# GATECH-EIC/BNS-GCN

Measured on AMD Instinct MI355X. Metric: training throughput (full-graph edges/s), reddit-shaped graphsage 3-layer h=256, sampling-rate=0.1, higher is better.
Workload: dtype fp32; 1 GPU; model=graphsage, dataset=reddit, n_layers=3, n_hidden=256, n_nodes=232965, n_edges=114756398, use_pp=True, partition=metis, parallelism=partition-parallel p1

## Files before the change

### bnsgcn_amd/models/context.py

```python
from __future__ import annotations

import torch

from ..graph.store import Partition
from ..ops.csr_torch import transpose_csr, merge_csr
from ..parallel.halo import partition_aggregate
from ..parallel.plan import EpochState, HaloPlan


def _inv_sqrt(x: torch.Tensor) -> torch.Tensor:
    return 1.0 / torch.sqrt(x.clamp_min(1.0))


def _inv(x: torch.Tensor) -> torch.Tensor:
    return 1.0 / x.clamp_min(1.0)


class GraphContext:
    def __init__(self, indptr, indices, in_deg, out_deg, device,
                 plan: HaloPlan | None = None, need_eperm: bool = True):
        dev = torch.device(device)
        self.plan = plan
        self.indptr = indptr.to(dev)
        self.indices = indices.to(dev)
        tip, tix, t_eperm = transpose_csr(self.indptr, self.indices,
                                          n_cols=self.indptr.numel() - 1
                                          if plan is None else plan.n_inner)
        self.t_indptr, self.t_indices = tip, tix
        self.t_eperm = t_eperm if need_eperm else None
        self.loss_rows: torch.Tensor | None = None
        self._rows_static: tuple | None = None
        self._rows_halo: tuple | None = None
        in_deg = in_deg.to(dev).float()
        out_deg = out_deg.to(dev).float()
        self.in_norm_inv = _inv_sqrt(in_deg)
        self.out_norm_inv = _inv_sqrt(out_deg)
        self.in_deg_inv = _inv(in_deg)
        self.n_rows = self.indptr.numel() - 1
        if dev.type == "cuda":
            from ..ops.functional import _worklist_of
            _worklist_of(self.indptr)
            _worklist_of(self.t_indptr)
        self._gat_cache: tuple[int, tuple] | None = None
        self._full_state: EpochState | None = None

    @classmethod
    def for_partition(cls, part: Partition, plan: HaloPlan, device,
                      need_eperm: bool = True) -> "GraphContext":
        return cls(torch.from_numpy(part.inner_indptr),
                   torch.from_numpy(part.inner_indices),
                   torch.from_numpy(part.in_deg),
                   torch.from_numpy(part.out_deg), device, plan=plan,
                   need_eperm=need_eperm)

    @classmethod
    def for_full_graph(cls, csr_indptr, csr_indices, in_deg, out_deg, device
                       ) -> "GraphContext":
        return cls(csr_indptr, csr_indices, in_deg, out_deg, device, plan=None)

    @property
    def inner_csrs(self):
        return (self.indptr, self.indices, self.t_indptr, self.t_indices)

    def aggregate(self, x: torch.Tensor, mode: str,
                  rows: torch.Tensor | None = None) -> torch.Tensor:
        if mode == "gcn":
            src, dst, halo_src = self.out_norm_inv, self.in_norm_inv, True
        elif mode == "mean":
            src, dst, halo_src = None, self.in_deg_inv, False
        else:
            raise ValueError(mode)
        if rows is not None:
            dst = dst[rows]
        if self.plan is None:
            from ..ops.functional import spmm_sum
            if rows is None:
                return spmm_sum(x, *self.inner_csrs, src_scale=src,
                                dst_scale=dst)
            ip, ix, tip, tix = self._rows_inner_csrs(rows)
            return spmm_sum(x, ip, ix, tip, tix, src_scale=src, dst_scale=dst)
        if rows is None:
            return partition_aggregate(x, self.plan, self.inner_csrs, src,
                                       dst, halo_src)
        import dataclasses
        st = self.plan.state
        hfip, hfix, hbip, hbix = self._rows_halo_csrs(rows, st)
        st_r = dataclasses.replace(st, halo_fwd_indptr=hfip,
                                   halo_fwd_indices=hfix,
                                   halo_bwd_indptr=hbip,
                                   halo_bwd_indices=hbix)
        ip, ix, tip, tix = self._rows_inner_csrs(rows)
        from ..parallel.halo import _PartitionAggregate
        return _PartitionAggregate.apply(x, self.plan, st_r, ip, ix, tip, tix,
                                         src, dst, halo_src)

    def _rows_inner_csrs(self, rows: torch.Tensor):
        from ..ops.csr_torch import gather_rows_csr
        if self._rows_static is None:
            ip, ix = gather_rows_csr(self.indptr, self.indices, rows)
            n_src = self.n_rows if self.plan is None else self.plan.n_inner
            tip, tix, _ = transpose_csr(ip, ix, n_src)
            if self.indptr.is_cuda:
                from ..ops.functional import _worklist_of
                _worklist_of(ip)
                _worklist_of(tip)
            self._rows_static = (ip, ix, tip, tix)
        return self._rows_static

    def _rows_halo_csrs(self, rows: torch.Tensor, st: EpochState):
        if self._rows_halo is not None and self._rows_halo[0] == st.epoch:
            ev = self._rows_halo[2]
            if ev is not None:
                cur = torch.cuda.current_stream()
                cur.wait_event(ev)
                for t in self._rows_halo[1]:
                    t.record_stream(cur)
                    wl = getattr(t, "_bns_worklist", None)
                    if wl is not None:
                        for w in wl:
                            w.record_stream(cur)
                self._rows_halo = (st.epoch, self._rows_halo[1], None)
            return self._rows_halo[1]
        out = self._build_rows_halo(rows, st)
        self._rows_halo = (st.epoch, out, None)
        return out
# ... 135 lines not shown
```

### bnsgcn_amd/ops/csr_torch.py

```python
from __future__ import annotations

import torch


def row_lengths(indptr: torch.Tensor) -> torch.Tensor:
    return indptr[1:] - indptr[:-1]


def transpose_csr(indptr: torch.Tensor, indices: torch.Tensor, n_cols: int
                  ) -> tuple[torch.Tensor, torch.Tensor, torch.Tensor]:
    device = indices.device
    n_rows = indptr.numel() - 1
    row = torch.repeat_interleave(torch.arange(n_rows, device=device, dtype=indices.dtype),
                                  row_lengths(indptr))
    eperm = torch.argsort(indices.long(), stable=True)
    indices_t = row[eperm]
    sorted_cols = indices[eperm]
    bounds = torch.arange(n_cols + 1, device=device, dtype=sorted_cols.dtype)
    indptr_t = torch.searchsorted(sorted_cols, bounds).to(indptr.dtype)
    return indptr_t, indices_t, eperm


import os

SEG = int(os.environ.get("BNSGCN_SEG", 512))
MAX_WAVES = int(os.environ.get("BNSGCN_MAX_WAVES", 131072))


def build_worklist(indptr: torch.Tensor, seg: int = None, max_waves: int = None
                   ) -> tuple[torch.Tensor, torch.Tensor, torch.Tensor, torch.Tensor]:
    seg = seg or SEG
    max_waves = max_waves or MAX_WAVES
    device = indptr.device
    deg = (indptr[1:] - indptr[:-1])
    n = deg.numel()
    nseg = torch.clamp((deg + (seg - 1)) // seg, min=1)
    total = int(nseg.sum())
    rows = torch.repeat_interleave(torch.arange(n, device=device), nseg)
    item_first = torch.cumsum(nseg, 0)
    item_first = torch.cat([torch.zeros(1, dtype=item_first.dtype, device=device),
                            item_first[:-1]])
    k = torch.arange(total, device=device) - item_first[rows]
    wbeg = indptr[rows] + k * seg
    wend = torch.minimum(wbeg + seg, indptr[rows + 1])
    split = nseg[rows] > 1
    wrow = torch.where(split, ~rows, rows).to(torch.int32)

    empty_rows = torch.nonzero(deg == 0, as_tuple=True)[0]
    atomic_rows = torch.nonzero(nseg > 1, as_tuple=True)[0]
    zero_rows = torch.cat([empty_rows, atomic_rows])
    keep = wend > wbeg
    wrow, wbeg, wend = wrow[keep], wbeg[keep], wend[keep]
    total = int(keep.sum())
    if total == 0:
        z = torch.zeros(0, dtype=torch.int32, device=device)
        return (z, wbeg, wend, torch.zeros(1, dtype=torch.int32, device=device),
                zero_rows)

    lens = (wend - wbeg)
    cum = torch.cumsum(torch.cat([torch.zeros(1, dtype=lens.dtype, device=device),
                                  lens]), 0)
    if total >= 1_000_000:
        max_waves = max(max_waves, 262144)
    n_waves = min(max_waves, max(8, total))
    n_waves = (n_waves + 7) // 8 * 8
    targets = (cum[-1] * torch.arange(n_waves + 1, device=device).double()
               / n_waves).to(cum.dtype)
    wave_start = torch.searchsorted(cum, targets).to(torch.int32)
    wave_start[0] = 0
    wave_start[-1] = total
    return (wrow.contiguous(), wbeg.contiguous(), wend.contiguous(),
            wave_start.contiguous(), zero_rows)


def merge_csr(ip1: torch.Tensor, ix1: torch.Tensor,
              ip2: torch.Tensor, ix2: torch.Tensor,
              col_offset2: int) -> tuple[torch.Tensor, torch.Tensor]:
    device = ix1.device
    n = ip1.numel() - 1
    l1 = row_lengths(ip1)
    l2 = row_lengths(ip2)
    ip = torch.zeros(n + 1, dtype=ip1.dtype, device=device)
    torch.cumsum(l1 + l2, 0, out=ip[1:])
    ix = torch.empty(int(ip[-1]), dtype=ix1.dtype, device=device)
    rows = torch.arange(n, device=device)
    if ix1.numel():
        r1 = torch.repeat_interleave(rows, l1)
        e1 = torch.arange(ix1.numel(), device=device)
        ix[ip[r1] + (e1 - ip1[r1])] = ix1
    if ix2.numel():
        r2 = torch.repeat_interleave(rows, l2)
        e2 = torch.arange(ix2.numel(), device=device)
        ix[ip[r2] + l1[r2] + (e2 - ip2[r2])] = (ix2 + col_offset2).to(ix1.dtype)
    return ip, ix


def gather_rows_csr(indptr: torch.Tensor, indices: torch.Tensor,
                    rows: torch.Tensor) -> tuple[torch.Tensor, torch.Tensor]:
    device = indices.device
    lens = row_lengths(indptr)[rows]
    new_indptr = torch.zeros(rows.numel() + 1, dtype=indptr.dtype, device=device)
    torch.cumsum(lens, 0, out=new_indptr[1:])
    total = int(new_indptr[-1])
    if total == 0:
        return new_indptr, torch.zeros(0, dtype=indices.dtype, device=device)
    starts = indptr[rows]
    pos = torch.arange(total, device=device)
    row_of_new_edge = torch.repeat_interleave(
        torch.arange(rows.numel(), device=device), lens)
    offset_in_row = pos - new_indptr[row_of_new_edge]
    src_edge = starts[row_of_new_edge] + offset_in_row
    return new_indptr, indices[src_edge]
```

### bnsgcn_amd/ops/functional.py

```python
from __future__ import annotations

import torch
from torch.autograd import Function

from . import reference as ref
from ._ext import get_ext, use_hip



def _worklist_of(indptr):
    wl = getattr(indptr, "_bns_worklist", None)
    if wl is None:
        from .csr_torch import build_worklist
        wl = build_worklist(indptr)
        indptr._bns_worklist = wl
    return wl


def spmm_sum_raw(indptr, indices, x, src_scale=None, dst_scale=None, out=None):
    if use_hip(x):
        wrow, wbeg, wend, wave_start, zero_rows = _worklist_of(indptr)
        acc = out is not None
        if not acc:
            out = torch.empty(indptr.numel() - 1, x.shape[1],
                              dtype=x.dtype, device=x.device)
            if zero_rows.numel():
                out.index_fill_(0, zero_rows, 0.0)
        return get_ext().spmm_sum(wrow, wbeg, wend, wave_start, indices, x,
                                  src_scale, dst_scale, out, acc)
    return ref.spmm_sum(indptr, indices, x, src_scale, dst_scale, out)


def spmm_edge_raw(indptr, indices, eweight, x, out=None, wperm=None):
    if use_hip(x):
        wrow, wbeg, wend, wstart, zero_rows = _worklist_of(indptr)
        acc = out is not None
        if not acc:
            out = torch.empty(indptr.numel() - 1, x.shape[1], x.shape[2],
                              dtype=x.dtype, device=x.device)
            if zero_rows.numel():
                out.index_fill_(0, zero_rows, 0.0)
        return get_ext().spmm_edge_sum(wrow, wbeg, wend, wstart, indptr,
                                       indices, eweight.contiguous(), wperm,
                                       x.contiguous(), out, acc)
    ew = eweight if wperm is None else eweight[wperm]
    return ref.spmm_edge_sum(indptr, indices, ew, x, out)


def sddmm_dot_raw(indptr, indices, a_dst, b_src):
    if use_hip(a_dst):
        wl = _worklist_of(indptr)[:4]
        return get_ext().sddmm_dot(*wl, indptr, indices,
                                   a_dst.contiguous(), b_src.contiguous())
    return ref.sddmm_dot(indptr, indices, a_dst, b_src)


def sddmm_add_raw(indptr, indices, el_src, er_dst, slope=-1.0):
    if use_hip(el_src):
        wl = _worklist_of(indptr)[:4]
        return get_ext().sddmm_add(*wl, indptr, indices,
                                   el_src.contiguous(), er_dst.contiguous(),
                                   slope)
    out = ref.sddmm_add(indptr, indices, el_src, er_dst)
    if slope >= 0:
        out = torch.nn.functional.leaky_relu(out, slope)
    return out


def segment_softmax_raw(indptr, logits):
    if use_hip(logits):
        return get_ext().segment_softmax(indptr, logits)
    return ref.segment_softmax(indptr, logits)


def segment_softmax_bwd_raw(indptr, alpha, grad_alpha):
    if use_hip(alpha):
        return get_ext().segment_softmax_backward(indptr, alpha, grad_alpha)
    return ref.segment_softmax_backward(indptr, alpha, grad_alpha)


def pack_rows_raw(x, idx, scale=None):
    if use_hip(x):
        return get_ext().pack_rows(x, idx, scale)
    return ref.pack_rows(x, idx, scale)


def scatter_add_rows_raw(out, idx, src, scale=None):
    if use_hip(out):
        get_ext().scatter_add_rows(out, idx, src, scale)
        return out
    return ref.scatter_add_rows(out, idx, src, scale)



class _SpMMSum(Function):

    @staticmethod
    def forward(ctx, x, indptr, indices, indptr_t, indices_t, src_scale, dst_scale):
        ctx.save_for_backward(indptr_t, indices_t, src_scale, dst_scale)
        return spmm_sum_raw(indptr, indices, x, src_scale, dst_scale)

    @staticmethod
    def backward(ctx, grad):
# ... 58 lines not shown
            gx_h = spmm_edge_raw(hbip, hbix, w_h, grad, wperm=heperm_t)
        if ctx.needs_input_grad[3]:
            gw_h = sddmm_dot_raw(hip_, hix_, grad, x_h)
        return (gx_in, gw_in, gx_h, gw_h) + (None,) * 10


def spmm_edge_sum2(x_in, w_in, x_h, w_h, inner_csrs5, halo_csrs5):
    return _SpMMEdge2.apply(x_in, w_in, x_h, w_h,
                            *inner_csrs5, *halo_csrs5)


class _SDDMMAdd(Function):

    @staticmethod
    def forward(ctx, el, er, indptr, indices, indptr_t, indices_t, eperm_t,
                slope):
        out = sddmm_add_raw(indptr, indices, el, er,
                            -1.0 if slope is None else float(slope))
        ctx.slope = slope
        if slope is not None:
            ctx.save_for_backward(indptr, indices, indptr_t, indices_t,
                                  eperm_t, out)
        else:
            ctx.save_for_backward(indptr, indices, indptr_t, indices_t,
                                  eperm_t)
        ctx.n_src, ctx.n_dst = el.shape[0], er.shape[0]
        return out

    @staticmethod
    def backward(ctx, grad):
        if ctx.slope is not None:
            indptr, indices, indptr_t, indices_t, eperm_t, out = ctx.saved_tensors
            grad = torch.where(out > 0, grad, grad * ctx.slope).contiguous()
        else:
            indptr, indices, indptr_t, indices_t, eperm_t = ctx.saved_tensors
            grad = grad.contiguous()
        g_el = g_er = None
        if use_hip(grad) and grad.shape[1] <= 8:
            e = get_ext()
            if ctx.needs_input_grad[0]:
                g_el = e.segment_sum_edges(*_worklist_of(indptr_t)[:4], eperm_t,
                                           grad, ctx.n_src)
            if ctx.needs_input_grad[1]:
                g_er = e.segment_sum_edges(*_worklist_of(indptr)[:4], None,
                                           grad, ctx.n_dst)
            return g_el, g_er, None, None, None, None, None, None
        if ctx.needs_input_grad[0]:
            g_el = torch.zeros(ctx.n_src, grad.shape[1], dtype=grad.dtype,
                               device=grad.device)
            g_el.index_add_(0, indices.long(), grad)
        if ctx.needs_input_grad[1]:
            g_er = torch.zeros(ctx.n_dst, grad.shape[1], dtype=grad.dtype,
                               device=grad.device)
            row = torch.repeat_interleave(
                torch.arange(ctx.n_dst, device=grad.device),
                indptr[1:] - indptr[:-1])
            g_er.index_add_(0, row, grad)
        return g_el, g_er, None, None, None, None, None, None


def sddmm_add(el, er, indptr, indices, indptr_t, indices_t, eperm_t,
              slope=None):
    return _SDDMMAdd.apply(el, er, indptr, indices, indptr_t, indices_t,
                           eperm_t, slope)


class _SegmentSoftmax(Function):
    @staticmethod
    def forward(ctx, logits, indptr):
        alpha = segment_softmax_raw(indptr, logits)
        ctx.save_for_backward(alpha, indptr)
        return alpha

    @staticmethod
    def backward(ctx, grad):
        alpha, indptr = ctx.saved_tensors
        return segment_softmax_bwd_raw(indptr, alpha, grad.contiguous()), None


def segment_softmax(logits, indptr):
    return _SegmentSoftmax.apply(logits, indptr)


import os as _os

_GEMM_MODE = _os.environ.get("BNSGCN_GEMM", "auto")


class _Linear(Function):

    @staticmethod
    def forward(ctx, x, weight, bias):
        ctx.save_for_backward(x, weight)
        ctx.has_bias = bias is not None
        if use_hip(x) and _GEMM_MODE == "hip":
            return get_ext().gemm_nt_bias(x, weight, bias)
        return torch.nn.functional.linear(x, weight, bias)

    @staticmethod
    def backward(ctx, grad):
        x, weight = ctx.saved_tensors
        grad = grad.contiguous()
        gx = gw = gb = None
        if use_hip(x):
            e = get_ext()
            if ctx.needs_input_grad[0]:
                gx = e.gemm_nn(grad, weight) if _GEMM_MODE == "hip" \
                    else grad @ weight
            if ctx.needs_input_grad[1]:
                gw = e.gemm_tn(grad, x)
            if ctx.has_bias and ctx.needs_input_grad[2]:
                return gx, gw, e.syncbn_stats(grad)[0]
        else:
            if ctx.needs_input_grad[0]:
                gx = grad @ weight
            if ctx.needs_input_grad[1]:
                gw = grad.t() @ x
        if ctx.has_bias and ctx.needs_input_grad[2]:
            gb = grad.sum(0)
        return gx, gw, gb


def linear(x, weight, bias=None):
    return _Linear.apply(x, weight, bias)


class _DropoutLinear(Function):

    @staticmethod
    def forward(ctx, x, weight, bias, keep, seed):
        x = x.contiguous()
        ctx.save_for_backward(x, weight)
        ctx.keep, ctx.seed = keep, seed
        ctx.has_bias = bias is not None
        return get_ext().gemm_nt_bias_drop(x, weight.contiguous(), bias,
                                           keep, seed)

    @staticmethod
    def backward(ctx, grad):
        x, weight = ctx.saved_tensors
        grad = grad.contiguous()
        e = get_ext()
        gw = gb = None
        if ctx.needs_input_grad[1]:
            gw = e.gemm_tn_drop(grad, x, ctx.keep, ctx.seed)
        if ctx.has_bias and ctx.needs_input_grad[2]:
            gb = e.syncbn_stats(grad)[0]
        return None, gw, gb, None, None


def dropout_linear(x, weight, bias, p: float, training: bool):
    if (training and p > 0.0 and use_hip(x) and x.dtype == torch.float32
            and not x.requires_grad):
        seed = int(torch.randint(0, 2**62, (1,)).item())
        return _DropoutLinear.apply(x, weight, bias, 1.0 - p, seed)
    return linear(dropout(x, p, training), weight, bias)


class _BiasAdd(Function):

    @staticmethod
    def forward(ctx, h, bias):
        return h + bias

    @staticmethod
    def backward(ctx, grad):
        gb = None
        if ctx.needs_input_grad[1]:
# ... 140 lines not shown
```

### bnsgcn_amd/ops/hip/kernels.hip

```cpp
#include <hip/hip_runtime.h>
#include <torch/extension.h>
#include <ATen/cuda/CUDAContext.h>
#include <c10/util/Optional.h>
#include <algorithm>
#include "common.h"
#include "gemm_tiled.h"

namespace {


DEV_INLINE void f4_axpy(float4& a, float ss, const float4 v) {
  a.x += ss * v.x; a.y += ss * v.y; a.z += ss * v.z; a.w += ss * v.w;
}

template <bool ACC, int SUBW>
__global__ __launch_bounds__(256) void spmm_sum_vec4_kernel(
    const int32_t* __restrict__ wrow, const int64_t* __restrict__ wbeg,
    const int64_t* __restrict__ wend, const int32_t* __restrict__ wave_start,
    const int32_t* __restrict__ indices, const float* __restrict__ x,
    const float* __restrict__ src_scale, const float* __restrict__ dst_scale,
    float* __restrict__ out, int f4) {
  const WorkList wl = {wrow, wbeg, wend, wave_start};
  const WaveItems wi = wave_items<SUBW>(wl);
  const int lane = wi.lane;
  const float4* __restrict__ x4 = reinterpret_cast<const float4*>(x);
  float4* __restrict__ out4 = reinterpret_cast<float4*>(out);

  for (int it = wi.beg; it < wi.end; ++it) {
    const WorkItem wk = work_item(wl, it);
    const float ds = dst_scale ? dst_scale[wk.row] : 1.0f;
    for (int f0 = 0; f0 < f4; f0 += 2 * SUBW) {
      const int fA = f0 + lane;
      const int fB = fA + SUBW;
      const bool hasA = fA < f4, hasB = fB < f4;
      float4 acc0 = {0.f, 0.f, 0.f, 0.f}, acc1 = {0.f, 0.f, 0.f, 0.f};
      for (int64_t e0 = wk.beg; e0 < wk.end; e0 += SUBW) {
        const Chunk ch = load_chunk<SUBW>(indices, src_scale, e0, wk.end, lane);
#pragma unroll 4
        for (int k = 0; k < ch.nv; ++k) {
          const int c = __shfl(ch.cid, k, SUBW);
          const float ss = src_scale ? __shfl(ch.ssc, k, SUBW) : 1.0f;
          const int64_t base = (int64_t)c * f4;
          if (hasA) f4_axpy(acc0, ss, x4[base + fA]);
          if (hasB) f4_axpy(acc1, ss, x4[base + fB]);
        }
      }
      const int64_t ob = (int64_t)wk.row * f4;
      if (hasA) store_row<ACC>(&out4[ob + fA], acc0, wk.atomic, ds);
      if (hasB) store_row<ACC>(&out4[ob + fB], acc1, wk.atomic, ds);
    }
  }
}

template <bool ACC, int G>
__global__ __launch_bounds__(256) void spmm_sum_narrow_kernel(
    const int32_t* __restrict__ wrow, const int64_t* __restrict__ wbeg,
    const int64_t* __restrict__ wend, const int32_t* __restrict__ wave_start,
    const int32_t* __restrict__ indices, const float* __restrict__ x,
    const float* __restrict__ src_scale, const float* __restrict__ dst_scale,
    float* __restrict__ out, int f4) {
  constexpr int NG = WAVE / G;
  const WorkList wl = {wrow, wbeg, wend, wave_start};
  const WaveItems wi = wave_items<WAVE>(wl);
  const int lane = wi.lane;
  const int g = lane / G, j = lane % G;
  const bool has = j < f4;
  const float4* __restrict__ x4 = reinterpret_cast<const float4*>(x);
  float4* __restrict__ out4 = reinterpret_cast<float4*>(out);

  for (int it = wi.beg; it < wi.end; ++it) {
    const WorkItem wk = work_item(wl, it);
    const float ds = dst_scale ? dst_scale[wk.row] : 1.0f;
    float4 acc = {0.f, 0.f, 0.f, 0.f};
    for (int64_t e0 = wk.beg; e0 < wk.end; e0 += WAVE) {
      const Chunk ch = load_chunk<WAVE>(indices, src_scale, e0, wk.end, lane);
#pragma unroll 4
      for (int k = 0; k < ch.nv; k += NG) {
        const int kk = k + g;
        const int c = __shfl(ch.cid, kk, WAVE);
        const float ss = src_scale ? __shfl(ch.ssc, kk, WAVE) : 1.0f;
        if (has && kk < ch.nv) f4_axpy(acc, ss, x4[(int64_t)c * f4 + j]);
      }
    }
#pragma unroll
    for (int off = G; off < WAVE; off <<= 1) {
      acc.x += __shfl_xor(acc.x, off, WAVE);
      acc.y += __shfl_xor(acc.y, off, WAVE);
      acc.z += __shfl_xor(acc.z, off, WAVE);
      acc.w += __shfl_xor(acc.w, off, WAVE);
    }
    if (g == 0 && has)
      store_row<ACC>(&out4[(int64_t)wk.row * f4 + j], acc, wk.atomic, ds);
  }
}

template <bool ACC>
__global__ __launch_bounds__(256) void spmm_sum_vec2_kernel(
    const int32_t* __restrict__ wrow, const int64_t* __restrict__ wbeg,
    const int64_t* __restrict__ wend, const int32_t* __restrict__ wave_start,
    const int32_t* __restrict__ indices, const float* __restrict__ x,
    const float* __restrict__ src_scale, const float* __restrict__ dst_scale,
    float* __restrict__ out, int f2) {
  const WorkList wl = {wrow, wbeg, wend, wave_start};
  const WaveItems wi = wave_items<WAVE>(wl);
  const int lane = wi.lane;
  const float2* __restrict__ x2 = reinterpret_cast<const float2*>(x);
  float2* __restrict__ out2 = reinterpret_cast<float2*>(out);
  for (int it = wi.beg; it < wi.end; ++it) {
    const WorkItem wk = work_item(wl, it);
    const float ds = dst_scale ? dst_scale[wk.row] : 1.0f;
    for (int f0 = 0; f0 < f2; f0 += 4 * WAVE) {
      float2 acc[4] = {{0.f, 0.f}, {0.f, 0.f}, {0.f, 0.f}, {0.f, 0.f}};
      for (int64_t e0 = wk.beg; e0 < wk.end; e0 += WAVE) {
        const Chunk ch = load_chunk<WAVE>(indices, src_scale, e0, wk.end, lane);
#pragma unroll 4
        for (int k = 0; k < ch.nv; ++k) {
          const int c = __shfl(ch.cid, k, WAVE);
          const float ss = src_scale ? __shfl(ch.ssc, k, WAVE) : 1.0f;
          const int64_t base = (int64_t)c * f2;
#pragma unroll
          for (int j = 0; j < 4; ++j) {
            const int f = f0 + j * WAVE + lane;
            if (f < f2) {
              const float2 v = x2[base + f];
              acc[j].x += ss * v.x;
              acc[j].y += ss * v.y;
            }
          }
        }
      }
      const int64_t ob = (int64_t)wk.row * f2;
#pragma unroll
// ... 1119 lines not shown
}

int env_int(const char* name, int dflt) {
  const char* e = getenv(name);
  return e ? atoi(e) : dflt;
}

struct WorkListArgs {
  WorkList wl;
  int n_waves;
};

WorkListArgs worklist_args(const at::Tensor& wrow, const at::Tensor& wbeg,
                           const at::Tensor& wend,
                           const at::Tensor& wave_start) {
  TORCH_CHECK(wrow.scalar_type() == at::kInt &&
                  wbeg.scalar_type() == at::kLong &&
                  wend.scalar_type() == at::kLong &&
                  wave_start.scalar_type() == at::kInt,
              "worklist: wrow/wave_start int32 and wbeg/wend int64 expected");
  for (const at::Tensor* t : {&wrow, &wbeg, &wend, &wave_start})
    TORCH_CHECK(t->is_cuda() && t->is_contiguous() &&
                    t->device() == wave_start.device(),
                "worklist arrays must be contiguous CUDA tensors on one "
                "device");
  TORCH_CHECK(wave_start.numel() >= 1 && wbeg.numel() == wrow.numel() &&
                  wend.numel() == wrow.numel(),
              "worklist: inconsistent array lengths (wrow ", wrow.numel(),
              ", wbeg ", wbeg.numel(), ", wend ", wend.numel(),
              ", wave_start ", wave_start.numel(), ")");
  const int n_waves = (int)wave_start.numel() - 1;
  TORCH_CHECK(n_waves % 8 == 0, "worklist: n_waves (", n_waves,
              ") must be a multiple of 8");
  return {{wrow.data_ptr<int32_t>(), wbeg.data_ptr<int64_t>(),
           wend.data_ptr<int64_t>(), wave_start.data_ptr<int32_t>()},
          n_waves};
}

template <typename K, typename... Args>
void launch_worklist(K kernel, const WorkListArgs& w, int subw,
                     Args... args) {
  hipLaunchKernelGGL(kernel, dim3(w.n_waves / (256 / subw)), dim3(256), 0,
                     at::cuda::getCurrentCUDAStream(), w.wl.row, w.wl.beg,
                     w.wl.end, w.wl.wave_start, args...);
}

at::Tensor spmm_sum(at::Tensor wrow, at::Tensor wbeg, at::Tensor wend,
                    at::Tensor wave_start, at::Tensor indices, at::Tensor x,
                    c10::optional<at::Tensor> src_scale,
                    c10::optional<at::Tensor> dst_scale,
                    at::Tensor out, bool acc) {
  check_f32(x, "x");
  check_f32(out, "out");
  TORCH_CHECK(indices.scalar_type() == at::kInt, "indices int32 expected");
  const WorkListArgs wl = worklist_args(wrow, wbeg, wend, wave_start);
  const int F = x.size(1);
  if (wrow.numel() == 0 || wl.n_waves <= 0) return out;
  static const int subw32_max = env_int("BNSGCN_SPMM_SUBW32_MAX", 32);
  static const int narrow_max =
      std::min(env_int("BNSGCN_SPMM_NARROW_MAX", 16), 16);
  auto launch = [&](auto kernel, int subw, int width) {
    launch_worklist(kernel, wl, subw, indices.data_ptr<int32_t>(),
                    x.data_ptr<float>(), opt_ptr(src_scale),
                    opt_ptr(dst_scale), out.data_ptr<float>(), width);
  };
  if (F % 4 == 0 && F / 4 <= std::min(narrow_max, subw32_max))
    launch(acc ? spmm_sum_narrow_kernel<true, 16>
               : spmm_sum_narrow_kernel<false, 16>, 64, F / 4);
  else if (F % 4 == 0 && F / 4 <= subw32_max)
    launch(acc ? spmm_sum_vec4_kernel<true, 32>
               : spmm_sum_vec4_kernel<false, 32>, 32, F / 4);
  else if (F % 4 == 0)
    launch(acc ? spmm_sum_vec4_kernel<true, 64>
               : spmm_sum_vec4_kernel<false, 64>, 64, F / 4);
  else if (F % 2 == 0)
    launch(acc ? spmm_sum_vec2_kernel<true> : spmm_sum_vec2_kernel<false>,
           64, F / 2);
  else
    launch(acc ? spmm_sum_scalar_kernel<true> : spmm_sum_scalar_kernel<false>,
           64, F);
  return out;
}

at::Tensor pack_rows(at::Tensor x, at::Tensor idx,
                     c10::optional<at::Tensor> scale) {
  check_f32(x, "x");
  TORCH_CHECK(idx.scalar_type() == at::kLong, "idx must be int64");
  const int n = idx.numel(), F = x.size(1);
  auto out = at::empty({n, F}, x.options());
  if (n == 0) return out;
  auto stream = at::cuda::getCurrentCUDAStream();
  const int64_t total = (int64_t)n * F;
  const int grid = std::min<int64_t>((total + 255) / 256, 4096);
  if (F % 4 == 0) {
    hipLaunchKernelGGL(pack_rows_vec4_kernel, dim3(grid), dim3(256), 0, stream,
                       x.data_ptr<float>(), idx.data_ptr<int64_t>(),
                       opt_ptr(scale), out.data_ptr<float>(), n, F / 4);
  } else {
    hipLaunchKernelGGL(pack_rows_kernel, dim3(grid), dim3(256), 0, stream,
                       x.data_ptr<float>(), idx.data_ptr<int64_t>(),
                       opt_ptr(scale), out.data_ptr<float>(), n, F);
  }
  return out;
}

void scatter_add_rows(at::Tensor out, at::Tensor idx, at::Tensor src,
                      c10::optional<at::Tensor> scale) {
  check_f32(out, "out");
  check_f32(src, "src");
  const int n = idx.numel(), F = out.size(1);
  if (n == 0) return;
  auto stream = at::cuda::getCurrentCUDAStream();
  const int64_t total = (int64_t)n * F;
  const int grid = std::min<int64_t>((total + 255) / 256, 4096);
  hipLaunchKernelGGL(scatter_add_rows_kernel, dim3(grid), dim3(256), 0, stream,
                     out.data_ptr<float>(), idx.data_ptr<int64_t>(),
                     src.data_ptr<float>(), opt_ptr(scale), n, F);
}

at::Tensor philox_keys(int64_t n, int64_t seed, int64_t epoch,
                       int64_t src_rank, int64_t dst_rank) {
  auto out = at::empty({n}, at::dtype(at::kLong).device(at::kCUDA));
  if (n == 0) return out;
  auto stream = at::cuda::getCurrentCUDAStream();
  const uint32_t sd = (((uint32_t)src_rank & 0xFFFF) << 16) |
                      ((uint32_t)dst_rank & 0xFFFF);
  hipLaunchKernelGGL(philox_keys_kernel, dim3((n + 255) / 256), dim3(256), 0,
                     stream, out.data_ptr<int64_t>(), (int)n,
                     (uint32_t)(seed & 0xFFFFFFFF),
                     (uint32_t)((seed >> 32) & 0xFFFFFFFF),
                     (uint32_t)(epoch & 0xFFFFFFFF), sd);
  return out;
}

at::Tensor syncbn_stats(at::Tensor x) {
  check_f32(x, "x");
  const int64_t n = x.size(0);
  const int F = x.size(1);
  auto out = at::zeros({2, F}, x.options());
  if (n == 0 || F == 0) return out;
  auto stream = at::cuda::getCurrentCUDAStream();
  const int row_chunks = (int)std::min<int64_t>((n + 255) / 256, 2048);
  dim3 grid((F + 255) / 256, row_chunks);
  hipLaunchKernelGGL(syncbn_stats_kernel, grid, dim3(256), 0, stream,
                     x.data_ptr<float>(), out.data_ptr<float>(), n, F,
                     row_chunks);
  return out;
}

std::vector<at::Tensor> ln_fwd(at::Tensor x, at::Tensor gamma,
                               at::Tensor beta, double eps, int64_t act) {
  check_f32(x, "x");
  check_f32(gamma, "gamma");
  check_f32(beta, "beta");
  const int64_t n = x.size(0);
  const int F = (int)x.size(1);
  TORCH_CHECK(F <= 64 * LN_MAX_K, "ln_fwd: F too large (", F, ")");
  auto y = at::empty_like(x);
  auto mean = at::empty({n}, x.options());
  auto rstd = at::empty({n}, x.options());
  auto stream = at::cuda::getCurrentCUDAStream();
  const int blocks = (int)std::min<int64_t>((n + 3) / 4, 32768);
  if (F % 4 == 0) {
    hipLaunchKernelGGL(
        ln_fwd_v4_kernel, dim3(std::max(blocks, 1)), dim3(256), 0, stream,
        reinterpret_cast<const float4*>(x.data_ptr<float>()),
// ... 339 lines not shown
  if (splitk > 1) {
    auto C = at::zeros({M, N}, A.options());
    const int k_slice = ((K + splitk - 1) / splitk + BK - 1) / BK * BK;
    grid.z = (K + k_slice - 1) / k_slice;
    hipLaunchKernelGGL(gemm_f32_kernel<true>, grid, dim3(256), 0, stream,
                       A.data_ptr<float>(), sAm, sAk, B.data_ptr<float>(), sBk,
                       sBn, opt_ptr(bias), C.data_ptr<float>(), M, N, K, k_slice);
    return C;
  }
  auto C = at::empty({M, N}, A.options());
  hipLaunchKernelGGL(gemm_f32_kernel<false>, grid, dim3(256), 0, stream,
                     A.data_ptr<float>(), sAm, sAk, B.data_ptr<float>(), sBk,
                     sBn, opt_ptr(bias), C.data_ptr<float>(), M, N, K, K);
  return C;
}

enum { GEMM_AUTO = 0, GEMM_OLD = 1, GEMM_TILED = 2 };

bool route_tiled(bns::GemmLayout layout, const at::Tensor& A,
                 const at::Tensor& B, int M, int N, int R, int64_t kernel) {
  TORCH_CHECK(kernel >= GEMM_AUTO && kernel <= GEMM_TILED, "bad kernel id");
  if (kernel == GEMM_OLD || M == 0 || N == 0 || R == 0) return false;
  if (kernel == GEMM_TILED) return true;
  if (!bns::gemm_tiled_aligned(layout, A, B, M, N, R) || R < 32) return false;
  auto pad = [](int64_t v, int64_t t) { return (v + t - 1) / t * t; };
  return 4 * pad(M, 128) * pad(N, 128) <= 5 * pad(M, BM) * pad(N, BN);
}

at::Tensor gemm_nt_bias(at::Tensor x, at::Tensor w,
                        c10::optional<at::Tensor> bias, int64_t kernel) {
  check_f32(x, "x"); check_f32(w, "w");
  const int M = x.size(0), K = x.size(1), N = w.size(0);
  TORCH_CHECK(w.size(1) == K, "shape mismatch");
  if (route_tiled(bns::GEMM_NT, x, w, M, N, K, kernel))
    return bns::gemm_tiled(bns::GEMM_NT, x, w, bias, M, N, K);
  return gemm_strided(x, K, 1, w, 1, K, bias, M, N, K);
}

at::Tensor gemm_nn(at::Tensor g, at::Tensor w, int64_t kernel) {
  check_f32(g, "g"); check_f32(w, "w");
  const int M = g.size(0), N = g.size(1), K = w.size(1);
  TORCH_CHECK(w.size(0) == N, "shape mismatch");
  if (route_tiled(bns::GEMM_NN, g, w, M, K, N, kernel))
    return bns::gemm_tiled(bns::GEMM_NN, g, w, c10::nullopt, M, K, N);
  return gemm_strided(g, N, 1, w, K, 1, c10::nullopt, M, K, N);
}

at::Tensor gemm_tn(at::Tensor g, at::Tensor x, int64_t kernel) {
  check_f32(g, "g"); check_f32(x, "x");
  const int M = g.size(0), N = g.size(1), K = x.size(1);
  TORCH_CHECK(x.size(0) == M, "shape mismatch");
  if (route_tiled(bns::GEMM_TN, g, x, N, K, M, kernel))
    return bns::gemm_tiled(bns::GEMM_TN, g, x, c10::nullopt, N, K, M);
  return gemm_strided(g, 1, N, x, K, 1, c10::nullopt, N, K, M);
}

at::Tensor gemm_nt_bias_drop(at::Tensor x, at::Tensor w,
                             c10::optional<at::Tensor> bias, double keep,
                             int64_t seed) {
  check_f32(x, "x"); check_f32(w, "w");
  const int M = x.size(0), K = x.size(1), N = w.size(0);
  TORCH_CHECK(w.size(1) == K, "shape mismatch");
  if (M == 0 || N == 0 || K == 0)
    return gemm_strided(x, K, 1, w, 1, K, bias, M, N, K);
  return bns::gemm_tiled(bns::GEMM_NT, x, w, bias, M, N, K, bns::DROP_A,
                         (float)keep, (uint64_t)seed);
}

at::Tensor gemm_tn_drop(at::Tensor g, at::Tensor x, double keep,
                        int64_t seed) {
  check_f32(g, "g"); check_f32(x, "x");
  const int M = g.size(0), N = g.size(1), K = x.size(1);
  TORCH_CHECK(x.size(0) == M, "shape mismatch");
  if (M == 0 || N == 0 || K == 0)
    return gemm_strided(g, 1, N, x, K, 1, c10::nullopt, N, K, M);
  return bns::gemm_tiled(bns::GEMM_TN, g, x, c10::nullopt, N, K, M,
                         bns::DROP_B, (float)keep, (uint64_t)seed);
}

}

PYBIND11_MODULE(TORCH_EXTENSION_NAME, m) {
  m.def("spmm_sum", &spmm_sum, "CSR SpMM sum with fused src/dst scales");
  m.def("pack_rows", &pack_rows, "gather rows + per-row scale");
  m.def("scatter_add_rows", &scatter_add_rows, "scatter-add rows + scale");
  m.def("philox_keys", &philox_keys, "BNS sampling keys (Philox4x32-10)");
  m.def("syncbn_stats", &syncbn_stats, "column sum + sum of squares");
  m.def("gemm_nt_bias", &gemm_nt_bias, "fp32 MFMA GEMM x@w^T+b",
        py::arg("x"), py::arg("w"), py::arg("bias"), py::arg("kernel") = 0);
  m.def("gemm_nn", &gemm_nn, "fp32 MFMA GEMM g@w", py::arg("g"),
        py::arg("w"), py::arg("kernel") = 0);
  m.def("gemm_tn", &gemm_tn, "fp32 MFMA GEMM g^T@x", py::arg("g"),
        py::arg("x"), py::arg("kernel") = 0);
  m.def("gemm_nt_bias_drop", &gemm_nt_bias_drop,
        "tiled GEMM dropout(x)@w^T+b, dropout fused into the operand load");
  m.def("gemm_tn_drop", &gemm_tn_drop,
        "tiled GEMM g^T@dropout(x), dropout fused into the operand load");
  m.def("sddmm_add", &sddmm_add, "GAT u_add_v SDDMM");
  m.def("segment_softmax", &segment_softmax, "edge softmax by dst segment");
  m.def("segment_softmax_backward", &segment_softmax_backward,
        "edge softmax backward");
  m.def("segment_softmax2", &segment_softmax2,
        "union softmax over two edge sets (split GAT block)");
  m.def("segment_softmax2_backward", &segment_softmax2_backward,
        "union softmax backward");
  m.def("spmm_edge_sum", &spmm_edge_sum, "multi-head edge-weighted SpMM");
  m.def("sddmm_dot", &sddmm_dot, "per-edge per-head dot (spmm_edge grad)");
  m.def("bincount_i32", &bincount_i32, "atomic int32 histogram");
  m.def("ln_fwd", &ln_fwd, "row LayerNorm forward (y, mean, rstd); "
        "act=1 fuses ReLU");
  m.def("ln_bwd", &ln_bwd, "row LayerNorm backward (dx, dgamma, dbeta)");
  m.def("dropout_apply", &dropout_apply,
        "mask-free dropout (splitmix64; same kernel fwd and bwd)");
  m.def("attn_project", &attn_project, "fused GAT el/er projections");
  m.def("attn_project_backward", &attn_project_backward,
        "fused GAT projection backward");
  m.def("segment_sum_edges", &segment_sum_edges,
        "segment sum of (permuted) edge values by CSR row");
}
```

Measured before the change: 4.073 billion edges/s.

## Add row-grouped SpMM that shares source-row loads across groups of destination rows

Builds a row-group sparse format in which each group of R consecutive destination rows gets one entry per distinct source column, with per-row uint8 multiplicities. A new HIP kernel reads each source feature row once per group and accumulates it into R row accumulators. The goal is fewer gathers of x when neighboring rows share neighbors, which is likely with METIS ordering. The format is used only when the entries-to-edges ratio is at or below a threshold, and by default only for the transposed (backward) CSR. The cost is extra preprocessing, R-times the accumulator registers, and wasted FLOPs on rows with zero weight.

```diff
diff --git a/bnsgcn_amd/models/context.py b/bnsgcn_amd/models/context.py
--- a/bnsgcn_amd/models/context.py
+++ b/bnsgcn_amd/models/context.py
@@ -37,10 +37,17 @@
         self.out_norm_inv = _inv_sqrt(out_deg)
         self.in_deg_inv = _inv(in_deg)
         self.n_rows = self.indptr.numel() - 1
+        self.rowgroup_ratio = (None, None)
         if dev.type == "cuda":
-            from ..ops.functional import _worklist_of
-            _worklist_of(self.indptr)
-            _worklist_of(self.t_indptr)
+            from ..ops import functional as BF
+            BF._worklist_of(self.indptr)
+            BF._worklist_of(self.t_indptr)
+            n_src = self.n_rows if plan is None else plan.n_inner
+            self.rowgroup_ratio = (
+                BF.attach_rowgroups(self.indptr, self.indices, n_src)
+                if BF.GROUP_FWD else None,
+                BF.attach_rowgroups(self.t_indptr, self.t_indices,
+                                    self.n_rows))
         self._gat_cache: tuple[int, tuple] | None = None
         self._full_state: EpochState | None = None
 
diff --git a/bnsgcn_amd/ops/csr_torch.py b/bnsgcn_amd/ops/csr_torch.py
--- a/bnsgcn_amd/ops/csr_torch.py
+++ b/bnsgcn_amd/ops/csr_torch.py
@@ -1,4 +1,6 @@
 from __future__ import annotations
+
+from typing import NamedTuple
 
 import torch
 
@@ -73,6 +75,70 @@
             wave_start.contiguous(), zero_rows)
 
 
+GROUP_R = int(os.environ.get("BNSGCN_SPMM_GROUP_R", 4))
+GSEG = int(os.environ.get("BNSGCN_GSEG", 1024))
+GROUP_W_MAX = 255
+
+
+class RowGroups(NamedTuple):
+    R: int
+    sched: tuple
+    ecol: torch.Tensor
+    ew: torch.Tensor
+    zero_rows: torch.Tensor
+    ratio: float
+
+
+def build_rowgroups(indptr: torch.Tensor, indices: torch.Tensor, n_cols: int,
+                    R: int = None, gseg: int = None, max_waves: int = None
+                    ) -> RowGroups:
+    R = R or GROUP_R
+    gseg = gseg or GSEG
+    device = indptr.device
+    n = indptr.numel() - 1
+    deg = indptr[1:] - indptr[:-1]
+    E = int(indices.numel())
+    n_groups = (n + R - 1) // R
+    row = torch.repeat_interleave(torch.arange(n, device=device), deg)
+    key = ((row // R) * n_cols + indices.long()) * R + row % R
+    del row
+    ukey, cnt = torch.unique(key, return_counts=True)
+    del key
+    pair, r = ukey // R, ukey % R
+    del ukey
+    pcol, inv = torch.unique_consecutive(pair, return_inverse=True)
+    egroup, ecol = pcol // n_cols, pcol % n_cols
+    n_pairs = pcol.numel()
+    nrep = (cnt + (GROUP_W_MAX - 1)) // GROUP_W_MAX
+    reps = torch.zeros(n_pairs, dtype=torch.int64, device=device)
+    reps.scatter_reduce_(0, inv, nrep, "amax", include_self=True)
+    first = torch.cumsum(reps, 0) - reps
+    n_ent = int(reps.sum())
+    ew = torch.zeros(n_ent, R, dtype=torch.uint8, device=device)
+    ew[first[inv], r] = cnt.clamp(max=GROUP_W_MAX).to(torch.uint8)
+    over = torch.nonzero(nrep > 1, as_tuple=True)[0]
+    if over.numel():
+        k = nrep[over] - 1
+        src = torch.repeat_interleave(over, k)
+        j = (torch.arange(src.numel(), device=device)
+             - torch.repeat_interleave(torch.cumsum(k, 0) - k, k) + 1)
+        ew[first[inv[src]] + j, r[src]] = (
+            (cnt[src] - GROUP_W_MAX * j).clamp(max=GROUP_W_MAX)
+            .to(torch.uint8))
+    ecol = torch.repeat_interleave(ecol, reps).to(torch.int32)
+    egroup = torch.repeat_interleave(egroup, reps)
+    gptr = torch.searchsorted(
+        egroup, torch.arange(n_groups + 1, device=device)).to(torch.int64)
+    wgroup, wbeg, wend, wave_start, zero_groups = build_worklist(
+        gptr, seg=gseg, max_waves=max_waves)
+    glen = gptr[1:] - gptr[:-1]
+    split = (glen > gseg)[torch.arange(n, device=device) // R]
+    zero_rows = torch.nonzero(split | (deg == 0), as_tuple=True)[0]
+    return RowGroups(R, (wgroup, wbeg, wend, wave_start), ecol.contiguous(),
+                     ew.contiguous(), zero_rows,
+                     n_ent / E if E else 1.0)
+
+
 def merge_csr(ip1: torch.Tensor, ix1: torch.Tensor,
               ip2: torch.Tensor, ix2: torch.Tensor,
               col_offset2: int) -> tuple[torch.Tensor, torch.Tensor]:
diff --git a/bnsgcn_amd/ops/functional.py b/bnsgcn_amd/ops/functional.py
--- a/bnsgcn_amd/ops/functional.py
+++ b/bnsgcn_amd/ops/functional.py
@@ -17,8 +17,40 @@
     return wl
 
 
+import os as _os
+
+_GROUP = _os.environ.get("BNSGCN_SPMM_GROUP", "1") != "0"
+GROUP_TAU = float(_os.environ.get("BNSGCN_SPMM_GROUP_TAU", 0.6))
+GROUP_FWD = _os.environ.get("BNSGCN_SPMM_GROUP_FWD", "0") == "1"
+
+
+def attach_rowgroups(indptr, indices, n_cols):
+    if not (_GROUP and indptr.is_cuda):
+        return None
+    from .csr_torch import build_rowgroups
+    rg = build_rowgroups(indptr, indices, n_cols)
+    keep = rg.ratio <= GROUP_TAU
+    if keep:
+        indptr._bns_rowgroups = rg
+    if _os.environ.get("BNSGCN_SPMM_GROUP_LOG") == "1":
+        print(f"rowgroup: R={rg.R} entries/edges {rg.ratio:.3f} "
+              f"({indices.numel()} edges) -> {'kept' if keep else 'dropped'}",
+              flush=True)
+    return rg.ratio
+
+
 def spmm_sum_raw(indptr, indices, x, src_scale=None, dst_scale=None, out=None):
     if use_hip(x):
+        rg = getattr(indptr, "_bns_rowgroups", None) if _GROUP else None
+        if rg is not None and x.shape[1] % 4 == 0 and x.shape[1] // 4 > 32:
+            acc = out is not None
+            if not acc:
+                out = torch.empty(indptr.numel() - 1, x.shape[1],
+                                  dtype=x.dtype, device=x.device)
+                if rg.zero_rows.numel():
+                    out.index_fill_(0, rg.zero_rows, 0.0)
+            return get_ext().spmm_sum_grouped(*rg.sched, rg.ecol, rg.ew, x,
+                                              src_scale, dst_scale, out, acc)
         wrow, wbeg, wend, wave_start, zero_rows = _worklist_of(indptr)
         acc = out is not None
         if not acc:
@@ -243,8 +275,6 @@
     return _SegmentSoftmax.apply(logits, indptr)
 
 
-import os as _os
-
 _GEMM_MODE = _os.environ.get("BNSGCN_GEMM", "auto")
 
 
diff --git a/bnsgcn_amd/ops/hip/kernels.hip b/bnsgcn_amd/ops/hip/kernels.hip
--- a/bnsgcn_amd/ops/hip/kernels.hip
+++ b/bnsgcn_amd/ops/hip/kernels.hip
@@ -48,6 +48,125 @@
       const int64_t ob = (int64_t)wk.row * f4;
       if (hasA) store_row<ACC>(&out4[ob + fA], acc0, wk.atomic, ds);
       if (hasB) store_row<ACC>(&out4[ob + fB], acc1, wk.atomic, ds);
+    }
+  }
+}
+
+template <int NW>
+DEV_INLINE void load_group_w(const uint32_t* __restrict__ p, uint32_t (&w)[NW]) {
+  if constexpr (NW == 1) {
+    w[0] = *p;
+  } else {
+    static_assert(NW == 2, "R in {4, 8}");
+    const uint2 t = *reinterpret_cast<const uint2*>(p);
+    w[0] = t.x; w[1] = t.y;
+  }
+}
+
+template <bool ACC, int R, int NV>
+__global__ __launch_bounds__(256) void spmm_sum_grouped_kernel(
+    const int32_t* __restrict__ wgroup, const int64_t* __restrict__ wbeg,
+    const int64_t* __restrict__ wend, const int32_t* __restrict__ wave_start,
+    const int32_t* __restrict__ ecol, const uint32_t* __restrict__ ew,
+    const float* __restrict__ x, const float* __restrict__ src_scale,
+    const float* __restrict__ dst_scale, float* __restrict__ out, int f4,
+    int n_rows) {
+  constexpr int NW = R / 4;
+  constexpr int U = 4;
+  const WorkList wl = {wgroup, wbeg, wend, wave_start};
+  const WaveItems wi = wave_items<WAVE>(wl);
+  const int lane = wi.lane;
+  const int it_beg = __builtin_amdgcn_readfirstlane(wi.beg);
+  const int it_end = __builtin_amdgcn_readfirstlane(wi.end);
+  const float4* __restrict__ x4 = reinterpret_cast<const float4*>(x);
+  float4* __restrict__ out4 = reinterpret_cast<float4*>(out);
+  const float4 zero4 = {0.f, 0.f, 0.f, 0.f};
+
+  for (int it = it_beg; it < it_end; ++it) {
+    const WorkItem wk = work_item(wl, it);
+    for (int f0 = 0; f0 < f4; f0 += NV * WAVE) {
+      int fi[NV];
+      bool has[NV];
+#pragma unroll
+      for (int v = 0; v < NV; ++v) {
+        fi[v] = f0 + v * WAVE + lane;
+        has[v] = fi[v] < f4;
+        if (!has[v]) fi[v] = f4 - 1;
+      }
+      float4 acc[NV][R];
+#pragma unroll
+      for (int v = 0; v < NV; ++v)
+#pragma unroll
+        for (int r = 0; r < R; ++r) acc[v][r] = zero4;
+      uint32_t seen[NW];
+#pragma unroll
+      for (int j = 0; j < NW; ++j) seen[j] = 0u;
+
+      auto accumulate = [&](int k, const float4 (&val)[NV], int ssc,
+                            const uint32_t (&wv)[NW]) {
+        const float ss = __int_as_float(__builtin_amdgcn_readlane(ssc, k));
+#pragma unroll
+        for (int j = 0; j < NW; ++j) {
+          const uint32_t w = (uint32_t)__builtin_amdgcn_readlane((int)wv[j], k);
+          seen[j] |= w;
+#pragma unroll
+          for (int b = 0; b < 4; ++b) {
+            const uint32_t cnt = (w >> (8 * b)) & 0xffu;
+            if (cnt != 0u) {
+              const float s = (float)cnt * ss;
+#pragma unroll
+              for (int v = 0; v < NV; ++v) f4_axpy(acc[v][4 * j + b], s, val[v]);
+            }
+          }
+        }
+      };
+
+      for (int64_t e0 = wk.beg; e0 < wk.end; e0 += WAVE) {
+        const int nv = (int)((wk.end - e0 < WAVE) ? (wk.end - e0) : WAVE);
+        int cid = 0, ssc = __float_as_int(1.0f);
+        uint32_t wv[NW];
+#pragma unroll
+        for (int j = 0; j < NW; ++j) wv[j] = 0u;
+        if (lane < nv) {
+          cid = ecol[e0 + lane];
+          if (src_scale) ssc = __float_as_int(src_scale[cid]);
+          load_group_w<NW>(ew + (e0 + lane) * NW, wv);
+        }
+        int k = 0;
+        for (; k + U <= nv; k += U) {
+          float4 val[U][NV];
+#pragma unroll
+          for (int u = 0; u < U; ++u) {
+            const int64_t base =
+                (int64_t)__builtin_amdgcn_readlane(cid, k + u) * f4;
+#pragma unroll
+            for (int v = 0; v < NV; ++v)
+              val[u][v] = x4[base + fi[v]];
+          }
+#pragma unroll
+          for (int u = 0; u < U; ++u) accumulate(k + u, val[u], ssc, wv);
+        }
+        for (; k < nv; ++k) {
+          float4 val[NV];
+          const int64_t base = (int64_t)__builtin_amdgcn_readlane(cid, k) * f4;
+#pragma unroll
+          for (int v = 0; v < NV; ++v) val[v] = x4[base + fi[v]];
+          accumulate(k, val, ssc, wv);
+        }
+      }
+
+#pragma unroll
+      for (int r = 0; r < R; ++r) {
+        const int row = wk.row * R + r;
+        if (((seen[r / 4] >> (8 * (r % 4))) & 0xffu) != 0u && row < n_rows) {
+          const float ds = dst_scale ? dst_scale[row] : 1.0f;
+          const int64_t ob = (int64_t)row * f4;
+#pragma unroll
+          for (int v = 0; v < NV; ++v)
+            if (has[v])
+              store_row<ACC>(&out4[ob + fi[v]], acc[v][r], wk.atomic, ds);
+        }
+      }
     }
   }
 }
@@ -1333,6 +1452,62 @@
   return out;
 }
 
+template <int R>
+void launch_grouped(const WorkListArgs& wl, bool acc, int f4,
+                    const at::Tensor& ecol, const at::Tensor& ew,
+                    const at::Tensor& x, const float* ss, const float* ds,
+                    at::Tensor& out) {
+  auto launch = [&](auto kernel) {
+    launch_worklist(kernel, wl, 64, ecol.data_ptr<int32_t>(),
+                    reinterpret_cast<const uint32_t*>(ew.data_ptr<uint8_t>()),
+                    x.data_ptr<float>(), ss, ds, out.data_ptr<float>(), f4,
+                    (int)out.size(0));
+  };
+  if (f4 > 64)
+    launch(acc ? spmm_sum_grouped_kernel<true, R, 2>
+               : spmm_sum_grouped_kernel<false, R, 2>);
+  else
+    launch(acc ? spmm_sum_grouped_kernel<true, R, 1>
+               : spmm_sum_grouped_kernel<false, R, 1>);
+}
+
+at::Tensor spmm_sum_grouped(at::Tensor wgroup, at::Tensor wbeg,
+                            at::Tensor wend, at::Tensor wave_start,
+                            at::Tensor ecol, at::Tensor ew, at::Tensor x,
+                            c10::optional<at::Tensor> src_scale,
+                            c10::optional<at::Tensor> dst_scale,
+                            at::Tensor out, bool acc) {
+  check_f32(x, "x");
+  check_f32(out, "out");
+  const WorkListArgs wl = worklist_args(wgroup, wbeg, wend, wave_start);
+  TORCH_CHECK(ecol.scalar_type() == at::kInt && ecol.is_cuda() &&
+                  ecol.is_contiguous(), "ecol: contiguous int32 expected");
+  TORCH_CHECK(ew.scalar_type() == at::kByte && ew.is_cuda() &&
+                  ew.is_contiguous() && ew.dim() == 2 &&
+                  ew.size(0) == ecol.numel(),
+              "ew: contiguous uint8 [n_entries, R] expected");
+  const int R = (int)ew.size(1);
+  const int F = x.size(1);
+  TORCH_CHECK(F % 4 == 0 && F / 4 > 32,
+              "spmm_sum_grouped covers F % 4 == 0 with F / 4 > 32, got F = ",
+              F);
+  TORCH_CHECK(out.dim() == 2 && out.size(1) == F, "out: [n_rows, F] expected");
+  if (src_scale.has_value())
+    TORCH_CHECK(src_scale->numel() == x.size(0), "src_scale: one per x row");
+  if (dst_scale.has_value())
+    TORCH_CHECK(dst_scale->numel() == out.size(0),
+                "dst_scale: one per out row");
+  if (wgroup.numel() == 0 || wl.n_waves <= 0) return out;
+  const float* ss = opt_ptr(src_scale);
+  const float* ds = opt_ptr(dst_scale);
+  switch (R) {
+    case 4: launch_grouped<4>(wl, acc, F / 4, ecol, ew, x, ss, ds, out); break;
+    case 8: launch_grouped<8>(wl, acc, F / 4, ecol, ew, x, ss, ds, out); break;
+    default: TORCH_CHECK(false, "spmm_sum_grouped: R must be 4 or 8, got ", R);
+  }
+  return out;
+}
+
 at::Tensor pack_rows(at::Tensor x, at::Tensor idx,
                      c10::optional<at::Tensor> scale) {
   check_f32(x, "x");
@@ -1838,6 +2013,8 @@
 
 PYBIND11_MODULE(TORCH_EXTENSION_NAME, m) {
   m.def("spmm_sum", &spmm_sum, "CSR SpMM sum with fused src/dst scales");
+  m.def("spmm_sum_grouped", &spmm_sum_grouped,
+        "row-group CSR SpMM sum with fused src/dst scales");
   m.def("pack_rows", &pack_rows, "gather rows + per-row scale");
   m.def("scatter_add_rows", &scatter_add_rows, "scatter-add rows + scale");
   m.def("philox_keys", &philox_keys, "BNS sampling keys (Philox4x32-10)");
```

Result: faster. 4.370 billion edges/s, median of 6 (+7.3%).
